# vpc-ccg/tksm

Measured on AMD Instinct MI355X. Metric: sequenced reads/s, higher is better.
Workload: dtype u8; 1 GPU; Bulk molecules, Badread error+qual model (nanopore2020, identity 84,99,5.5), 24 x 128 Mb random genome, FASTQ; kind=bulk, mean_len=1000, length_distribution=normal(1000, 200), compute_qual=True, contexts_in_flight_per_gpu=3

## Files before the change

### tksm_amd/csrc/kernels.hip

```cpp
#include "kernels.h"
#include "loop_filter.h"
#include <type_traits>

namespace tk {

#define DEV __device__ __forceinline__

constexpr int BIG = 1 << 28;
DEV bool is_inf(int v) { return v >= (1 << 27); }

struct Ph4 { uint32_t x, y, z, w; };
enum { ST_ID = 0, ST_PAD = 1, ST_IDENT = 2, ST_DRAW = 3, ST_ALNPOS = 4, ST_QUAL = 5, ST_TAIL = 6 };

DEV Ph4 philox(uint64_t seed, uint64_t read, uint32_t stream, uint32_t n) {
    uint32_t c0 = (uint32_t)read, c1 = (uint32_t)(read >> 32), c2 = stream, c3 = n;
    uint32_t k0 = (uint32_t)seed, k1 = (uint32_t)(seed >> 32);
#pragma unroll
    for (int r = 0; r < 10; r++) {
        const unsigned long long p0 = (unsigned long long)0xD2511F53u * c0, p1 = (unsigned long long)0xCD9E8D57u * c2;
        const uint32_t h0 = (uint32_t)(p0 >> 32), l0 = (uint32_t)p0, h1 = (uint32_t)(p1 >> 32), l1 = (uint32_t)p1;
        uint32_t n0 = h1 ^ c1 ^ k0, n2 = h0 ^ c3 ^ k1;
        c0 = n0; c1 = l1; c2 = n2; c3 = l0;
        k0 += 0x9E3779B9u; k1 += 0xBB67AE85u;
    }
    return Ph4{c0, c1, c2, c3};
}

DEV uint8_t base_char(int code) { return (uint8_t)((0x54474341u >> (8 * (code & 3))) & 0xff); }
DEV int code_of(uint8_t c) { return c == 'A' ? 0 : c == 'C' ? 1 : c == 'G' ? 2 : c == 'T' ? 3 : -1; }
DEV uint8_t upper(uint8_t c) { return (c >= 'a' && c <= 'z') ? (uint8_t)(c - 32) : c; }
DEV uint8_t comp(uint8_t c) {
    return c == 'A' ? 'T' : c == 'C' ? 'G' : c == 'G' ? 'C' : c == 'T' ? 'A' : c;
}

template <int CTRL, int ROW_MASK> DEV int dpp_mov(int old, int src) { return __builtin_amdgcn_update_dpp(old, src, CTRL, ROW_MASK, 0xf, false); }
constexpr int DPP_WAVE_SHL1 = 0x130, DPP_WAVE_SHR1 = 0x138;
#define TKSM_DPP_SCAN(OP, IDENT, x)                         \
    x = OP(x, dpp_mov<0x111, 0xf>(IDENT, x));               \
    x = OP(x, dpp_mov<0x112, 0xf>(IDENT, x));               \
    x = OP(x, dpp_mov<0x114, 0xf>(IDENT, x));               \
    x = OP(x, dpp_mov<0x118, 0xf>(IDENT, x));               \
    x = OP(x, dpp_mov<0x142, 0xa>(IDENT, x));               \
    x = OP(x, dpp_mov<0x143, 0xc>(IDENT, x));
DEV int scan_min_incl(int x, int) { TKSM_DPP_SCAN(min, 0x7fffffff, x) return x; }
DEV int scan_max_incl(int x, int) { TKSM_DPP_SCAN(max, (int)0x80000000, x) return x; }
DEV int add_i32(int a, int b) { return a + b; }
DEV int scan_add_incl(int x, int) { TKSM_DPP_SCAN(add_i32, 0, x) return x; }
DEV uint32_t scan_umax_incl(uint32_t x) {
#define TKSM_UMAX_STEP(C, R) x = max(x, (uint32_t)dpp_mov<C, R>(0, (int)x));
    TKSM_UMAX_STEP(0x111, 0xf) TKSM_UMAX_STEP(0x112, 0xf) TKSM_UMAX_STEP(0x114, 0xf) TKSM_UMAX_STEP(0x118, 0xf) TKSM_UMAX_STEP(0x142, 0xa) TKSM_UMAX_STEP(0x143, 0xc)
#undef TKSM_UMAX_STEP
    return x;
}
DEV int prefix_small(int v, int& total) {
    const unsigned long long b0 = __ballot(v & 1), b1 = __ballot(v & 2), b2 = __ballot(v & 4);
    const int e0 = (int)__builtin_amdgcn_mbcnt_hi((uint32_t)(b0 >> 32), __builtin_amdgcn_mbcnt_lo((uint32_t)b0, 0u));
    const int e1 = (int)__builtin_amdgcn_mbcnt_hi((uint32_t)(b1 >> 32), __builtin_amdgcn_mbcnt_lo((uint32_t)b1, 0u));
    const int e2 = (int)__builtin_amdgcn_mbcnt_hi((uint32_t)(b2 >> 32), __builtin_amdgcn_mbcnt_lo((uint32_t)b2, 0u));
    total = __popcll(b0) + 2 * __popcll(b1) + 4 * __popcll(b2);
    return e0 + 2 * e1 + 4 * e2;
}

DEV void wave_sync() {
    __builtin_amdgcn_fence(__ATOMIC_RELEASE, "wavefront");
    __builtin_amdgcn_wave_barrier();
    __builtin_amdgcn_fence(__ATOMIC_ACQUIRE, "wavefront");
}

DEV uint32_t lo32(unsigned long long v) { return (uint32_t)v; }
DEV uint32_t hi32(unsigned long long v) { return (uint32_t)(v >> 32); }
DEV unsigned long long mk64(uint32_t hi, uint32_t lo) { return ((unsigned long long)hi << 32) | lo; }
DEV uint32_t alignbit(uint32_t hi, uint32_t lo, uint32_t s) { return __builtin_amdgcn_alignbit(hi, lo, s); }
constexpr uint32_t TA = 0xF0u, TB = 0xCCu, TC = 0xAAu;
#define BOOL3(expr) ((uint32_t)((expr) & 0xFFu))
template <uint32_t TT> DEV uint32_t bool3(uint32_t x, uint32_t y, uint32_t z) { return __builtin_amdgcn_bitop3_b32(x, y, z, TT); }
template <uint32_t TT> DEV unsigned long long bool3(unsigned long long x, unsigned long long y, unsigned long long z) {
    return mk64(bool3<TT>(hi32(x), hi32(y), hi32(z)), bool3<TT>(lo32(x), lo32(y), lo32(z)));
}
DEV unsigned long long funnel128(unsigned long long x0, unsigned long long x1, int s) {
    const bool a = (s & 32) != 0;
    const uint32_t b = (uint32_t)s & 31u;
    const uint32_t y0 = a ? hi32(x0) : lo32(x0), y1 = a ? lo32(x1) : hi32(x0), y2 = a ? hi32(x1) : lo32(x1);
    return mk64(alignbit(y2, y1, b), alignbit(y1, y0, b));
}

DEV double sqrt_inrange(double x) {
    const double y = __builtin_amdgcn_rsq(x);
    double g = x * y, h = 0.5 * y;
    const double r = __builtin_fma(-h, g, 0.5);
    g = __builtin_fma(g, r, g); h = __builtin_fma(h, r, h);
    double d = __builtin_fma(-g, g, x);
    g = __builtin_fma(d, h, g);
    d = __builtin_fma(-g, g, x);
    return __builtin_fma(d, h, g);
}
DEV double rcp_refined(double b) {
    double y = __builtin_amdgcn_rcp(b);
    double r = __builtin_fma(-b, y, 1.0);
    y = __builtin_fma(y, r, y);
    r = __builtin_fma(-b, y, 1.0);
    return __builtin_fma(y, r, y);
}
DEV double div_inrange(double a, double b, double yb) {
    const double q = a * yb;
    const double r = __builtin_fma(-b, q, a);
    return __builtin_fma(r, yb, q);
}

DEV uint8_t ref_base(const RefView& R, uint64_t g) {
// ... 843 lines not shown
            dirty |= code < 0;
            const unsigned long long lo = __ballot(valid && (code & 1)), hi = __ballot(valid && (code & 2));
            if (lane == q - q0) { mylo = lo; myhi = hi; }
        }
        if (q0 + lane < fw_r) { ulonglong2 v; v.x = mylo; v.y = myhi; *reinterpret_cast<ulonglong2*>(fpl + 2 * (q0 + lane)) = v; }
    }
    const bool slow = __ballot(dirty) != 0ull;
    if (lane == 0) {
        ReadState S;
        S.errors = 0.0; S.target = target; S.est = 0.0; S.change_count = 0; S.n_base = 0; S.aln_no = 0;
        S.resume_src = -1; S.resume_j = 0; S.stage = 0; S.pending = 0; S.slow = slow ? 1 : 0; S.early = 0;
        S.st_draws = 0; S.st_aligns = 0; S.job = 0; S.raw_len = raw_len; S.res_mt = 0; S.res_cols = 0; S.res_fail = 0; S.pad3 = 0;
        FB.state[r] = S;
        O.status[r] |= status;
        if (slow) { const uint32_t idx = atomicAdd(&FB.counters[CNT_SLOW], 1u); FB.slow_list[idx] = (uint32_t)r; }
        else if (FB.early_hist) atomicAdd(&FB.early_hist[(blockIdx.x & 63u) * 256u + early_bin(L, target)], 1u);
    }
}

DEV void finish_read(const BatchView& B, const SimParams& P, const SimBuffers& O, uint64_t r, int raw_len, int out_len,
                     double identity, uint32_t status, int st_draws, int st_changes, int st_aligns, int L, int st_newlen,
                     int st_strim, int st_etrim, double errors, double target, int lane) {
    if (lane != 0) return;
    if (O.tail_len && !P.quirk_perfect) raw_len -= (int)O.tail_len[r];
    const long long h = pct_hundredths(identity);
    const uint32_t idl = B.ids[2 * r + 1];
    uint64_t rec = 1 + 36 + 8 + ndigits((unsigned)out_len) + 19 + ndigits((unsigned)raw_len) + 15 +
                   ndigits((unsigned long long)(h / 100)) + 3 + 14 + idl + 1;
    rec += (uint64_t)out_len + 1;
    if (P.fastq) rec += 2 + (uint64_t)out_len + 1;
    O.out_len[r] = (uint32_t)out_len;
    O.identity[r] = identity;
    O.rec_len[r] = rec;
    O.status[r] |= status;
    if (O.istats) {
        int32_t* s = O.istats + 16 * r;
        s[0] = st_draws; s[1] = st_changes; s[2] = st_aligns; s[3] = L; s[4] = st_newlen;
        s[5] = st_strim; s[6] = st_etrim; s[7] = (int32_t)status;
        O.dstats[2 * r] = errors; O.dstats[2 * r + 1] = target;
    }
}

DEV uint32_t draw_slot(const uint4& A, int jj) {
    const uint32_t w = (jj >> 1) == 0 ? A.x : (jj >> 1) == 1 ? A.y : (jj >> 1) == 2 ? A.z : A.w;
    return (w >> (16 * (jj & 1))) & 0xffffu;
}

DEV uint32_t planar1(uint32_t a) { return (a & 1u) | ((a >> 1) << 5); }
DEV uint32_t planar2(uint32_t a, uint32_t b) { return (a & 1u) | ((b & 1u) << 1) | ((a >> 1) << 5) | ((b >> 1) << 6); }
DEV uint4 random_change_enc(int kidx, int k, uint32_t type, uint32_t pos, uint32_t base4, uint32_t side, uint32_t r3) {
    uint32_t e[8];
#pragma unroll
    for (int j = 0; j < 8; j++) {
        const uint32_t kc = j < k ? (uint32_t)(kidx >> (2 * (k - 1 - j))) & 3u : 0u;
        uint32_t v = (1u << 12) | planar1(kc);
        if ((uint32_t)j == pos)
            v = type == 0 ? 0x8000u | (1u << 12) | planar1((kc + r3) & 3u)
              : type == 1 ? 0x8000u | (2u << 12) | (side ? planar2(kc, base4) : planar2(base4, kc))
                          : 0x8000u;
        e[j] = j < k ? v : 0u;
    }
    return make_uint4(e[0] | (e[1] << 16), e[2] | (e[3] << 16), e[4] | (e[5] << 16), e[6] | (e[7] << 16));
}

struct SlotEval { uint32_t am, lens; uint32_t e[4]; };
DEV SlotEval eval_draw(const uint16_t* nb, int k, int i, const uint4& A, bool acc) {
    SlotEval r;
    r.am = 0; r.lens = 0;
    r.e[0] = A.x | 0x80008000u; r.e[1] = A.y | 0x80008000u; r.e[2] = A.z | 0x80008000u; r.e[3] = A.w | 0x80008000u;
    if (acc) {
#pragma unroll
        for (int jj = 0; jj < 8; jj++) {
            if (jj < k) {
                const uint32_t e = draw_slot(A, jj);
                if ((e >> 15) && (nb[i + jj] & 0x8000u) == 0) r.am |= 1u << jj;
                r.lens |= ((e >> 12) & 7u) << (3 * jj);
            }
        }
    }
    return r;
}

DEV int joined_len(const uint16_t* nb, int p0, int n, int lane) {
    int m = 0;
    for (int q = 0; q < n; q += 64) {
        const int p = q + lane;
        const int len = p < n ? slot_len(nb[p0 + p]) : 0;
        int total;
        (void)prefix_small(len, total);
        m += total;
    }
    return m;
}

DEV void join_out(const uint8_t* frag, const uint16_t* nb, int n, uint8_t* out_seq, int lo, int hi, int lane) {
    int base = 0;
    for (int q = 0; q < n; q += 64) {
        const int p = q + lane;
        uint32_t code = 0; int len = 0; uint8_t orig = 0;
        if (p < n) { code = nb[p]; len = slot_len(code); orig = frag[p]; }
        int total;
        const int off = base + prefix_small(len, total);
        const uint32_t syms = code ? code & 0x3ffu : planar1((uint32_t)orig);
        for (int x2 = 0; x2 < len; x2++) { const int c = off + x2; if (c >= lo && c < hi) out_seq[c - lo] = base_char((int)(((syms >> x2) & 1u) | (((syms >> (5 + x2)) & 1u) << 1))); }
        base += total;
    }
}

#ifndef TKSM_LOOP_N
#define TKSM_LOOP_N 16
#define TKSM_LOOP_K 3
#endif
constexpr int LOOP_N = TKSM_LOOP_N, LOOP_K = TKSM_LOOP_K;
__global__ __launch_bounds__(64) __attribute__((amdgpu_num_vgpr(128))) void k_loop(ErrModelView EM, SimParams P, FastBuffers FB, const uint32_t* __restrict__ order,
                                              uint32_t begin, uint32_t count, int Wl, int from_jobs, uint32_t c0, uint32_t c1) {
#ifndef TKSM_ABLATE
    __builtin_amdgcn_s_setprio(2);
#endif
    uint32_t* lf = reinterpret_cast<uint32_t*>(lds_raw);
    const int lane = threadIdx.x;
    const uint32_t widx = blockIdx.x * 64u + (uint32_t)lane;
    bool act = widx < count;
    uint32_t r = 0, rc = 0;
    if (act) {
        if (!from_jobs) { r = order[begin + widx]; rc = (begin + widx) / FB.rs; }
        else {
            const uint32_t target = FB.prefix[c0] + widx;
            uint32_t lo2 = c0, hi2 = c1 - 1;
            while (lo2 < hi2) { const uint32_t mid = (lo2 + hi2 + 1) >> 1; if (FB.prefix[mid] <= target) lo2 = mid; else hi2 = mid - 1; }
            r = FB.prev_meta[4ull * (FB.base_prev[lo2] + (target - FB.prefix[lo2]))];
            rc = lo2;
        }
    }
    ReadState* sp = FB.state + r;
    ReadState S{};
    if (act) S = *sp;
    act = act && S.stage == 0 && !S.slow && !S.early;
    const int k = EM.k;
    const int L = S.raw_len + 2 * k;
    const uint32_t* f2 = frag2_row(FB, r);
    for (int w = 0; w < Wl; w += 16) {
        uint4 v[4];
#pragma unroll
        for (int q = 0; q < 4; q++) v[q] = *reinterpret_cast<const uint4*>(f2 + min(w + 4 * q, Wl - 4));
#pragma unroll
        for (int q = 0; q < 4; q++) {
            const int ww = min(w + 4 * q, Wl - 4);
            lf[(ww + 0) * 64 + lane] = v[q].x; lf[(ww + 1) * 64 + lane] = v[q].y; lf[(ww + 2) * 64 + lane] = v[q].z; lf[(ww + 3) * 64 + lane] = v[q].w;
        }
    }
    uint32_t* lfb = lf + (size_t)Wl * 64;
    {
        uint4 v[4];
#pragma unroll
        for (int q = 0; q < 4; q++) v[q] = EM.pt0b[q * 64 + lane];
#pragma unroll
        for (int q = 0; q < 4; q++) *reinterpret_cast<uint4*>(lfb + 4 * (q * 64 + lane)) = v[q];
    }
    __syncthreads();
    const uint16_t* lfe = reinterpret_cast<const uint16_t*>(lfb);
    uint16_t* gnb = nb_row(FB, r);
    const uint64_t g = P.first_read + (uint64_t)r * P.stride;
    const double frag_len = (double)L, target = S.target;
    const double rcp_len = rcp_refined(act ? frag_len : 1.0);
    double errors = S.errors;
    int change_count = S.change_count;
    uint32_t n = S.n_base, aln_no = S.aln_no;
    int resume_j = S.resume_j, st_draws = S.st_draws;
    double est_keep = S.est;
    if (act && S.pending == 1) {
        const uint32_t mt = S.res_mt, cols = S.res_cols;
        if (S.res_fail) {
            sp->slow = 1;
            atomicAdd(&FB.counters[CNT_EXIT + EXIT_BAND_LOOP], 1u);
            FB.slow_list[atomicAdd(&FB.counters[CNT_SLOW], 1u)] = r;
            act = false;
        } else {
            const double ident = cols ? (double)mt / (double)cols : 0.0;
            if (L <= 1000) errors = (1.0 - ident) * frag_len;
            else {
                const double estimated = (1.0 - ident) * frag_len;
                const double weight = 1000.0 / frag_len;
                errors = estimated * weight + errors * (1.0 - weight);
            }
            aln_no++;
        }
    }
    const uint32_t kmer_range = (uint32_t)(L - k);
    const long long loop_limit = 100ll * L;
    const uint32_t kmask = (1u << (2 * k)) - 1u;
    int cc25 = change_count % 25;
    enum { RUN = 0, NEED_ALN = 1, DONE = 2, IDLE = 3 };
    int st = act ? RUN : IDLE;
#ifdef TKSM_ABLATE
    if (P.ablate == 33) st = IDLE;
#endif
    const bool use_tab = EM.type != 0 && EM.alt0_noop;
    while (__ballot(st == RUN) != 0ull) {
        if (st != RUN) continue;
        const uint32_t navail = (uint32_t)max(0ll, min((long long)LOOP_N, loop_limit - (long long)n));
        uint32_t mask = 0u;
        {
            uint32_t dwv[LOOP_N], kxv[LOOP_N];
#pragma unroll
            for (int b = 0; b < LOOP_N; b++) {
                const Ph4 d = philox(P.seed, g, ST_DRAW, n + (uint32_t)b);
                const int di1 = (int)__umulhi(d.x, kmer_range);
                dwv[b] = d.y;
                const int w = di1 >> 4, o = di1 & 15;
#ifdef TKSM_ABLATE
                const bool abl_lds = P.ablate == 35 || P.ablate == 36;
                const uint32_t hi = (abl_lds || w < Wl) ? lf[min(w, Wl - 1) * 64 + lane] : f2[w], lo = (abl_lds || w + 1 < Wl) ? lf[min(w + 1, Wl - 1) * 64 + lane] : f2[w + 1];
#else
                const uint32_t hi = w < Wl ? lf[w * 64 + lane] : f2[w], lo = w + 1 < Wl ? lf[(w + 1) * 64 + lane] : f2[w + 1];
#endif
                kxv[b] = (uint32_t)(mk64(hi, lo) >> (64 - 2 * o - 2 * k)) & kmask;
            }
            uint32_t ev[LOOP_N];
#pragma unroll
            for (int b = 0; b < LOOP_N; b++) ev[b] = lfe[tklf::loop_filter_key(kxv[b])];
            uint32_t sure = 0u, und = 0u;
#pragma unroll
            for (int b = 0; b < LOOP_N; b++) {
                const int c = tklf::loop_filter_classify(ev[b], dwv[b]);
                sure |= c == tklf::DRAW_CHANGE ? 1u << b : 0u;
                und |= c == tklf::DRAW_UNDECIDED ? 1u << b : 0u;
            }
            if (!use_tab) { sure = (1u << LOOP_N) - 1u; und = 0u; }
#ifdef TKSM_ABLATE
            const bool abl_t0 = P.ablate == 34 || P.ablate == 36;
            if (abl_t0 && use_tab) { sure = 0u; und = (1u << LOOP_N) - 1u; }
#endif
            uint32_t t0v[LOOP_N];
#pragma unroll
            for (int b = 0; b < LOOP_N; b++) {
                const uint32_t off = (und >> b) & 1u ? kxv[b] << 2 : 0u;
#ifdef TKSM_ABLATE
                t0v[b] = abl_t0 ? 0xCF000000u : *reinterpret_cast<const uint32_t*>(reinterpret_cast<const char*>(EM.pt0) + off);
#else
                t0v[b] = *reinterpret_cast<const uint32_t*>(reinterpret_cast<const char*>(EM.pt0) + off);
#endif
            }
#pragma unroll
            for (int b = 0; b < LOOP_N; b++) mask |= !(dwv[b] < t0v[b]) ? 1u << b : 0u;
            mask = (sure | (und & mask)) & ((1u << navail) - 1u);
        }
        int di[LOOP_K], kidx[LOOP_K];
        uint32_t bj[LOOP_K], dw[LOOP_K];
        bool rest;
        {
            uint32_t mm = mask;
#pragma unroll
            for (int j = 0; j < LOOP_K; j++) {
                bj[j] = mm ? (uint32_t)__builtin_ctz(mm) : (uint32_t)LOOP_N;
                mm &= mm - 1u;
                const uint32_t bb = min(bj[j], (uint32_t)LOOP_N - 1u);
                const Ph4 d = philox(P.seed, g, ST_DRAW, n + bb);
                dw[j] = d.y;
                di[j] = (int)__umulhi(d.x, kmer_range);
                const int w = di[j] >> 4, o = di[j] & 15;
                const uint32_t hi = w < Wl ? lf[w * 64 + lane] : f2[w], lo = w + 1 < Wl ? lf[(w + 1) * 64 + lane] : f2[w + 1];
                kidx[j] = (int)((uint32_t)(mk64(hi, lo) >> (64 - 2 * o - 2 * k)) & kmask);
            }
            rest = mm != 0u;
        }
        int cls[LOOP_K];
        uint4 seg[LOOP_K];
        int nab[LOOP_K];
#pragma unroll
        for (int j = 0; j < LOOP_K; j++) { seg[j] = EM.pseg[kidx[j]]; nab[j] = EM.max_alts; }
        if (!EM.uniform_nalts) {
#pragma unroll
            for (int j = 0; j < LOOP_K; j++) nab[j] = (int)EM.nalts[kidx[j]];
        }
        int sbase[LOOP_K];
        uint4 th0[LOOP_K], th1[LOOP_K];
        struct __attribute__((packed, aligned(4))) W5 { uint32_t v[5]; };
        W5 nbw[LOOP_K];
#pragma unroll
        for (int j = 0; j < LOOP_K; j++) {
            const bool have = bj[j] < (uint32_t)LOOP_N;
            cls[j] = !have ? 0 : EM.type == 0 ? 2 : (dw[j] < seg[j].x ? (EM.alt0_noop ? 0 : 3) : 1);
            sbase[j] = 8 * ((dw[j] < seg[j].y ? 0 : 1) + (dw[j] < seg[j].z ? 0 : 1) + (dw[j] < seg[j].w ? 0 : 1));
            const uint4* c4 = reinterpret_cast<const uint4*>(EM.cdf32 + (cls[j] == 1 ? (size_t)kidx[j] * 32 + sbase[j] : (size_t)0));
            th0[j] = c4[0]; th1[j] = c4[1];
            const uint16_t* gp = cls[j] != 0 ? gnb + (di[j] & ~1) : FB.st_nb;
            nbw[j] = *reinterpret_cast<const W5*>(gp);
        }
        uint4 alt[LOOP_K];
#pragma unroll
        for (int j = 0; j < LOOP_K; j++) {
            size_t at = 0;
            if (cls[j] == 1 || cls[j] == 3) {
                const int na = nab[j];
                int a2 = 0;
                if (cls[j] == 1) {
                    const uint32_t w = dw[j];
                    a2 = sbase[j];
                    a2 += !(w < th0[j].x) ? 1 : 0; a2 += !(w < th0[j].y) ? 1 : 0; a2 += !(w < th0[j].z) ? 1 : 0; a2 += !(w < th0[j].w) ? 1 : 0;
                    a2 += !(w < th1[j].x) ? 1 : 0; a2 += !(w < th1[j].y) ? 1 : 0; a2 += !(w < th1[j].z) ? 1 : 0; a2 += !(w < th1[j].w) ? 1 : 0;
                    a2 = min(a2, na);
                }
                if (a2 == na) cls[j] = 2;
                else if (a2 == 0 && EM.alt0_noop) cls[j] = 0;
                else at = (size_t)kidx[j] * EM.max_alts + a2;
            }
            alt[j] = EM.alts_enc[at];
        }
        const uint32_t n0 = n;
        const uint32_t end = rest ? bj[LOOP_K - 1] + 1u : navail;
        uint32_t wrote = 0u;
        auto top_of_iteration = [&](double& est) -> bool {
            est = 1.0 - div_inrange(errors, frag_len, rcp_len);
            if ((double)change_count > 0.9 * frag_len || est <= target) { st = DONE; st_draws = (int)n; return false; }
            if ((long long)n + 1 > loop_limit) { st = DONE; st_draws = (int)loop_limit; return false; }
            return true;
        };
#pragma unroll
        for (int j = 0; j <= LOOP_K; j++) {
            if (st != RUN) break;
            double est = est_keep;
            if (j == LOOP_K || bj[j] >= (uint32_t)LOOP_N) {
                if (n - n0 < end) { if (!top_of_iteration(est)) break; n = n0 + end; }
                if (!rest && navail < (uint32_t)LOOP_N) (void)top_of_iteration(est);
                break;
            }
            if (resume_j == 0 && !top_of_iteration(est)) break;
            n = n0 + bj[j];
            if (cls[j] != 0) {
                uint4 A = alt[j];
                if (cls[j] == 2) {
                    const Ph4 d2 = philox(P.seed, g, ST_DRAW, n0 + bj[j]);
                    const uint32_t dzj = d2.z, dvj = d2.w;
                    const uint32_t type = __umulhi(dzj, 3u), pos = __umulhi(dvj, (uint32_t)k);
                    const uint32_t base4 = dvj & 3u, side = (dvj >> 2) & 1u;
                    const uint32_t r3 = (((dzj & 0xffffu) * 3u) >> 16) + 1u;
                    const uint32_t kc = ((uint32_t)kidx[j] >> (2 * (k - 1 - (int)pos))) & 3u;
                    const uint32_t v = type == 0 ? 0x8000u | (1u << 12) | planar1((kc + r3) & 3u)
                                     : type == 1 ? 0x8000u | (2u << 12) | (side ? planar2(kc, base4) : planar2(base4, kc))
                                                 : 0x8000u;
                    const uint32_t w = v << (16 * (pos & 1u)), which = pos >> 1;
                    A = make_uint4(which == 0 ? w : 0u, which == 1 ? w : 0u, which == 2 ? w : 0u, which == 3 ? w : 0u);
                }
                uint32_t dm = ((A.x >> 15) & 1u) | ((A.x >> 31) << 1) | (((A.y >> 15) & 1u) << 2) | ((A.y >> 31) << 3) |
                              (((A.z >> 15) & 1u) << 4) | ((A.z >> 31) << 5) | (((A.w >> 15) & 1u) << 6) | ((A.w >> 31) << 7);
                dm &= ((1u << k) - 1u) & ~((1u << resume_j) - 1u);
                if (dm) {
                    bool stale = false;
#pragma unroll
                    for (int j2 = 0; j2 < LOOP_K; j2++) if (j2 < j) stale |= ((wrote >> j2) & 1u) && abs(di[j] - di[j2]) < k;
                    if (stale) nbw[j] = *reinterpret_cast<const W5*>(gnb + (di[j] & ~1));
                    const double f15 = est * sqrt_inrange(est);
                    const int odd = di[j] & 1;
                    int stop_at = -1;
                    while (dm) {
                        const int jj = __builtin_ctz(dm);
                        dm &= dm - 1u;
                        const int ent = jj + odd, wi = ent >> 1;
                        const uint32_t cw2 = wi == 0 ? nbw[j].v[0] : wi == 1 ? nbw[j].v[1] : wi == 2 ? nbw[j].v[2] : wi == 3 ? nbw[j].v[3] : nbw[j].v[4];
                        if (((cw2 >> (16 * (ent & 1))) & 0x8000u) == 0u) {
                            const uint32_t e = draw_slot(A, jj);
                            gnb[di[j] + jj] = (uint16_t)(e | 0x8000u);
                            wrote |= 1u << j;
                            change_count++;
                            const int len_j = (int)((e >> 12) & 7u);
                            errors += (double)(len_j < 2 ? 1 : len_j - 1) * f15;
                            if (++cc25 == 25) { cc25 = 0; stop_at = jj; dm = 0u; }
                        }
                    }
                    if (stop_at >= 0) {
                        st = NEED_ALN;
                        if (stop_at + 1 < k) { resume_j = stop_at + 1; est_keep = est; }
                        else { resume_j = 0; n++; }
                        break;
                    }
                }
            }
            resume_j = 0;
            n++;
        }
    }
    int st_aligns = S.st_aligns;
    uint32_t job = 0;
    {
        bool need = st == NEED_ALN;
        unsigned long long todo = __ballot(need);
        while (todo) {
            const int leader = __builtin_ctzll(todo);
            const uint32_t lrc = (uint32_t)__shfl((int)rc, leader, 64);
            const unsigned long long grp = __ballot(need && rc == lrc);
            uint32_t base = 0;
            if (lane == leader) base = FB.base_cur[lrc] + atomicAdd(&FB.job_cnt[lrc * 32u], (uint32_t)__popcll(grp));
            base = (uint32_t)__shfl((int)base, leader, 64);
            if (need && rc == lrc) { job = base + (uint32_t)__popcll(grp & ((1ull << lane) - 1ull)); need = false; }
            todo &= ~grp;
        }
    }
    if (st == NEED_ALN) {
        st_aligns++;
        uint32_t p0 = 0, nrows = (uint32_t)L;
        if (L > 1000) {
            uint32_t r2 = r;
            asm volatile("" : "+v"(r2));
            p0 = __umulhi(philox(P.seed, P.first_read + (uint64_t)r2 * P.stride, ST_ALNPOS, aln_no).x, (uint32_t)(L - 1000 + 1));
            nrows = 1000u;
        }
        *reinterpret_cast<uint4*>(FB.job_meta + 4ull * job) = make_uint4(r, p0, nrows, 0u);
    }
    if (st == NEED_ALN || st == DONE) {
        sp->errors = errors; sp->est = est_keep; sp->change_count = change_count; sp->n_base = n; sp->aln_no = aln_no;
        sp->resume_src = -1; sp->resume_j = (int16_t)resume_j; sp->st_draws = st_draws; sp->st_aligns = st_aligns;
        sp->pending = st == NEED_ALN ? 1 : 0;
        sp->job = job;
        sp->stage = st == NEED_ALN ? 0 : 3;
        if (st == DONE) {
// ... 299 lines not shown
        const uint32_t pjob = FB.base_prev[lo2] + (target - FB.prefix[lo2]);
        r = (uint64_t)__builtin_amdgcn_readfirstlane((int)FB.prev_meta[4ull * pjob]) & 0xffffffffull;
        pos = lo2 * FB.rs;
    }
    ReadState S = FB.state[r];
    if (S.stage == 2 || S.slow) return;
    if (S.stage == 0) return;
    uint16_t* gnb = nb_row(FB, r);
    const int per_wave = STATE_IN_HBM ? lds_ncap + 128 : lds_lcap * 3 + lds_ncap + 128;
    uint8_t* lds_wave = lds_raw + (size_t)wave * per_wave;
    uint8_t* frag = STATE_IN_HBM ? frag_row(FB, r) : lds_wave;
    uint16_t* nb = STATE_IN_HBM ? gnb : reinterpret_cast<uint16_t*>(lds_wave + lds_lcap);
    uint8_t* aux = STATE_IN_HBM ? lds_wave : lds_wave + 3 * (size_t)lds_lcap;
    const int k = EM.k;
    const uint64_t g = P.first_read + r * P.stride;
    const int raw_len = __builtin_amdgcn_readfirstlane(S.raw_len);
    const int L = raw_len + 2 * k;
    const uint64_t slot = O.slot_off[r];
    const int cap = __builtin_amdgcn_readfirstlane((int)((O.slot_off[r + 1] - slot) >> 1));
    uint8_t* out_seq = O.scratch + slot;
    uint8_t* out_qual = out_seq + cap;
    if (!STATE_IN_HBM) {
        const uint8_t* gfrag0 = frag_row(FB, r);
        for (int t = lane * 4; t < L; t += 256) *reinterpret_cast<uint32_t*>(frag + t) = *reinterpret_cast<const uint32_t*>(gfrag0 + t);
        for (int t = lane * 2; t < L; t += 128) *reinterpret_cast<uint32_t*>(nb + t) = *reinterpret_cast<const uint32_t*>(gnb + t);
    }
    wave_sync();
    uint32_t status = 0;
    const double frag_len = (double)L;
    const double errors = S.errors;
    const double target = S.target;
    const int change_count = __builtin_amdgcn_readfirstlane(S.change_count), st_draws = __builtin_amdgcn_readfirstlane(S.st_draws);
    int st_aligns = __builtin_amdgcn_readfirstlane(S.st_aligns);
    double identity = 1.0;

    int start_trim, end_trim;
    {
        int v1 = lane < k ? slot_len(nb[lane]) : 0, v2 = lane < k ? slot_len(nb[L - k + lane]) : 0;
        (void)prefix_small(v1, start_trim);
        (void)prefix_small(v2, end_trim);
    }
    const int jcap = min(lds_ncap, cap);
    const int m = joined_len(nb, 0, L, lane);
    int lo = start_trim, hi = end_trim == 0 ? 0 : m - end_trim;
    lo = min(lo, m); hi = max(hi, lo);
    if (m > jcap) { status |= 1; lo = hi = 0; }
    const int out_len = hi - lo;
    const bool want_q = P.compute_q && m > 0 && !(status & 1);
    if (want_q) {
        const uint32_t mt = S.res_mt, cols = S.res_cols, fail = S.res_fail;
        if (fail) { go_slow(FB, r, lane, EXIT_BAND_ERR); return; }
        identity = cols ? (double)mt / (double)cols : 0.0;
        const uint32_t rc1 = pos / FB.rs;
        const uint8_t* gp = FB.prev_popd + FB.geo_prev[rc1].popd_off + (size_t)(S.job - FB.base_prev[rc1]) * FB.geo_prev[rc1].ncap;
        wave_sync();
        uint8_t* popd = aux + 16;
        for (int t = lane; t < m; t += 64) popd[t] = gp[t];
        wave_sync();
        const int margins = (QM.kmer_size - 1) / 2;
        const uint32_t hmask = (uint32_t)QM.n_slots - 1u;
        for (int i2 = lo + lane; i2 < hi; i2 += 64) {
#ifdef TKSM_ABLATE
            if (P.ablate == 40) { out_qual[i2 - lo] = 40; continue; }
#endif
            const int d = max(0, max(margins - i2, i2 + margins - (m - 1)));
            int row = -1; uint32_t roff = 0, rcnt = 0;
            auto probe = [&](uint64_t key) {
                uint32_t sl = (uint32_t)qs_hash(key) & hmask;
#ifdef TKSM_ABLATE
                if (P.ablate == 41) { row = (int)(sl & 1023u); roff = 0u; rcnt = 1u; return; }
#endif
                for (;;) {
                    const uint4 e = QM.ent[sl];
                    const uint64_t kk = ((uint64_t)e.y << 32) | e.x;
                    if (kk == key) { row = (int)sl; roff = e.z; rcnt = e.w; break; }
                    if (kk == 0) break;
                    sl = (sl + 1) & hmask;
                }
            };
            if (margins <= 4) {
                const int ob = 16 + i2 - 4, sh = ob & 3;
                const uint32_t* aw = reinterpret_cast<const uint32_t*>(aux) + (ob >> 2);
                const uint32_t w0 = aw[0], w1 = aw[1], w2 = aw[2];
                const uint32_t b0 = __builtin_amdgcn_alignbyte(w1, w0, sh), b1 = __builtin_amdgcn_alignbyte(w2, w1, sh), b2 = w2 >> (8 * sh);
                auto byte_at = [&](int j) -> uint32_t { return j < 4 ? (b0 >> (8 * j)) & 255u : j < 8 ? (b1 >> (8 * (j - 4))) & 255u : b2 & 255u; };
                uint64_t K[5]; int ln[5];
                K[0] = byte_at(4) & 3u; ln[0] = 1;
#pragma unroll
                for (int h = 1; h <= 4; h++) {
                    const uint32_t bl = byte_at(4 - h);
                    const int ddl = (int)(bl >> 2), ddr = (int)(byte_at(3 + h) >> 2);
                    ln[h] = ln[h - 1] + 2 + ddl + ddr;
                    const bool fits = ln[h] <= 29;
                    const int sl_ = fits ? 2 * (1 + ddl) : 0, sr_ = fits ? 2 * (1 + ddl + ln[h - 1]) : 0, so_ = fits ? 2 * (ln[h] - 1) : 0;
                    const int dl2 = fits ? 2 * ddl : 0, dr2 = fits ? 2 * ddr : 0;
                    K[h] = (uint64_t)(bl & 3u) | (((1ull << dl2) - 1ull) << 2) | (K[h - 1] << sl_) | (((1ull << dr2) - 1ull) << sr_) |
                           ((uint64_t)(byte_at(4 + h) & 3u) << so_);
                }
                const int hmax = margins - d;
                bool pend = true;
#pragma unroll
                for (int h = 4; h >= 0; h--) {
                    const bool tryit = pend && h <= hmax;
                    if (__ballot(tryit) == 0ull) continue;
                    if (tryit && ln[h] <= 29) { probe(K[h] | ((uint64_t)ln[h] << 58)); pend = row < 0; }
#ifdef TKSM_ABLATE
                    if (P.ablate == 44) { if (row < 0) row = (int)(K[h] & 1023u); pend = false; }
                    if (P.ablate == 45 && h == 3) { if (row < 0) row = (int)(K[h] & 1023u); pend = false; }
#endif
                }
            } else {
                int s0 = i2 - margins + d, e0 = i2 + margins - d;
                for (;;) {
                    uint64_t key = 0; int len = 0; bool ok = true;
                    for (int x2 = s0; x2 <= e0; x2++) {
                        if (x2 > s0) {
                            const int dd = popd[x2 - 1] >> 2;
                            if (len + dd > 29) { ok = false; break; }
                            key |= ((1ull << (2 * dd)) - 1ull) << (2 * len); len += dd;
                        }
                        if (len >= 29) { ok = false; break; }
                        key |= (uint64_t)(popd[x2] & 3) << (2 * len); len++;
                    }
                    if (ok) probe(key | ((uint64_t)len << 58));
                    if (row >= 0 || s0 == e0) break;
                    s0++; e0--;
                }
            }
            uint8_t q = 0;
#ifdef TKSM_ABLATE
            if (P.ablate == 42) { out_qual[i2 - lo] = (uint8_t)(33 + (row & 31)); continue; }
            if (P.ablate == 43 && row >= 0) {
                const uint32_t w = (uint32_t)i2 * 2654435761u;
                const uint32_t a2 = QM.guide[(size_t)row * 64 + (w >> 26)] & 0x7fu;
                out_qual[i2 - lo] = (uint8_t)(33 + QM.pairs[roff + min(a2, rcnt - 1u)].y); continue;
            }
#endif
            if (row >= 0) {
                const uint32_t w = philox(P.seed, g, ST_QUAL, (uint32_t)i2).x;
                uint32_t a2 = QM.guide[(size_t)row * 64 + (w >> 26)];
                if (QM.guide_direct && (a2 & 0x80u)) q = (uint8_t)(a2 & 0x7fu);
                else {
                    uint2 pr = QM.pairs[roff + a2];
                    while (a2 + 1 < rcnt && !(w < pr.x)) { a2++; pr = QM.pairs[roff + a2]; }
                    q = (uint8_t)pr.y;
                }
            }
            out_qual[i2 - lo] = (uint8_t)(q + 33);
        }
    } else {
        identity = 1.0 - errors / frag_len;
    }
    join_out(frag, nb, L, out_seq, lo, hi, lane);
    if (P.quirk_perfect) identity = 1.0;
    finish_read(B, P, O, r, P.quirk_perfect ? out_len : raw_len, out_len, identity, status, st_draws, change_count, st_aligns, L, m,
                start_trim, end_trim, errors, target, lane);
    if (lane == 0) FB.state[r].stage = 2;
}

__global__ void k_collect_unfinished(FastBuffers FB, uint64_t n_reads) {
    const uint64_t r = (uint64_t)blockIdx.x * blockDim.x + threadIdx.x;
    if (r >= n_reads) return;
    ReadState S = FB.state[r];
    if (S.stage != 2 && !S.slow) {
        FB.state[r].slow = 1;
        const uint32_t idx = atomicAdd(&FB.counters[CNT_SLOW], 1u);
        FB.slow_list[idx] = (uint32_t)r;
    }
}

DEV uint32_t range_of_job(const FastBuffers& FB, uint32_t job0) {
    uint32_t rng = 0, hi2 = FB.n_ranges - 1;
    while (rng < hi2) { const uint32_t mid = (rng + hi2 + 1) >> 1; if (FB.base_cur[mid] <= job0) rng = mid; else hi2 = mid - 1; }
    return rng;
}
__global__ __launch_bounds__(64) void k_qjobs(FastBuffers FB, int k, uint32_t count) {
    const int lane = threadIdx.x;
    const uint32_t widx = blockIdx.x * 64u + (uint32_t)lane;
    bool need = widx < count;
    uint32_t r = 0, rc = 0, job = 0;
    if (need) { const uint2 e = FB.defer_list[widx]; r = e.x; rc = e.y; }
    need = need && FB.state[r].stage == 3 && !FB.state[r].slow;
    const bool mine = need;
    unsigned long long todo = __ballot(need);
    while (todo) {
        const int leader = __builtin_ctzll(todo);
        const uint32_t lrc = (uint32_t)__shfl((int)rc, leader, 64);
        const unsigned long long grp = __ballot(need && rc == lrc);
        uint32_t base = 0;
        if (lane == leader) base = FB.base_cur[lrc] + atomicAdd(&FB.job_cnt[lrc * 32u], (uint32_t)__popcll(grp));
        base = (uint32_t)__shfl((int)base, leader, 64);
        if (need && rc == lrc) { job = base + (uint32_t)__popcll(grp & ((1ull << lane) - 1ull)); need = false; }
        todo &= ~grp;
    }
    if (mine) {
        ReadState* sp = FB.state + r;
        const uint32_t L = (uint32_t)(sp->raw_len + 2 * k);
        *reinterpret_cast<uint4*>(FB.job_meta + 4ull * job) = make_uint4(r, 0u, L | 0x80000000u, 0u);
        sp->resume_src = -1; sp->pending = 1; sp->stage = 1; sp->job = job;
    }
}

DEV int wave_max(int v) {
#pragma unroll
    for (int o = 32; o > 0; o >>= 1) v = max(v, __shfl_xor(v, o, 64));
    return v;
}
DEV void list_append(uint32_t* list, uint32_t* counter, bool want, uint32_t job, int lane) {
    const unsigned long long wm = __ballot(want);
    if (!wm) return;
    uint32_t base = 0;
    if (lane == 0) base = atomicAdd(counter, (uint32_t)__popcll(wm));
    base = __shfl(base, 0, 64);
    if (want) list[base + (uint32_t)__popcll(wm & ((1ull << lane) - 1ull))] = job;
}


constexpr uint32_t ENT_EMPTY = 0xF0000000u;
constexpr int BACKLOG_DRAIN = 20;
struct AlnJobF {
    bool act; int p0, n;
    const uint16_t* nb;
// ... 993 lines not shown
```

Before: 15.68 million reads/s.

## Use bitop3 XOR in Philox, flat SWAR quality keys, and cheaper join loops

Adds a templated Philox that emits the three-input XOR through the gfx950 bitop3 intrinsic from a chosen round onward, used for draw and quality RNG. Replaces the nested per-level quality-key construction with a SWAR byte-prefix flat key builder that takes 32-bit, 64-bit or a nested fallback path chosen per wave. Simplifies joined_len to one strided accumulation plus a single wave scan, and unrolls the join_out per-slot writes with a ballot guard. These aim to cut ALU work in hot RNG, quality and join code, at the cost of more code paths and subtle key-equivalence risk.

```diff
diff --git a/tksm_amd/csrc/kernels.hip b/tksm_amd/csrc/kernels.hip
--- a/tksm_amd/csrc/kernels.hip
+++ b/tksm_amd/csrc/kernels.hip
@@ -1,5 +1,6 @@
 #include "kernels.h"
 #include "loop_filter.h"
+#include "qs_keys.h"
 #include <type_traits>
 
 namespace tk {
@@ -12,19 +13,23 @@
 struct Ph4 { uint32_t x, y, z, w; };
 enum { ST_ID = 0, ST_PAD = 1, ST_IDENT = 2, ST_DRAW = 3, ST_ALNPOS = 4, ST_QUAL = 5, ST_TAIL = 6 };
 
-DEV Ph4 philox(uint64_t seed, uint64_t read, uint32_t stream, uint32_t n) {
+template <int LANE_FROM>
+DEV Ph4 philox_t(uint64_t seed, uint64_t read, uint32_t stream, uint32_t n) {
     uint32_t c0 = (uint32_t)read, c1 = (uint32_t)(read >> 32), c2 = stream, c3 = n;
     uint32_t k0 = (uint32_t)seed, k1 = (uint32_t)(seed >> 32);
 #pragma unroll
     for (int r = 0; r < 10; r++) {
         const unsigned long long p0 = (unsigned long long)0xD2511F53u * c0, p1 = (unsigned long long)0xCD9E8D57u * c2;
         const uint32_t h0 = (uint32_t)(p0 >> 32), l0 = (uint32_t)p0, h1 = (uint32_t)(p1 >> 32), l1 = (uint32_t)p1;
-        uint32_t n0 = h1 ^ c1 ^ k0, n2 = h0 ^ c3 ^ k1;
+        uint32_t n0, n2;
+        if (r >= LANE_FROM) { n0 = __builtin_amdgcn_bitop3_b32(h1, c1, k0, 0x96u); n2 = __builtin_amdgcn_bitop3_b32(h0, c3, k1, 0x96u); }
+        else { n0 = h1 ^ c1 ^ k0; n2 = h0 ^ c3 ^ k1; }
         c0 = n0; c1 = l1; c2 = n2; c3 = l0;
         k0 += 0x9E3779B9u; k1 += 0xBB67AE85u;
     }
     return Ph4{c0, c1, c2, c3};
 }
+DEV Ph4 philox(uint64_t seed, uint64_t read, uint32_t stream, uint32_t n) { return philox_t<10>(seed, read, stream, n); }
 
 DEV uint8_t base_char(int code) { return (uint8_t)((0x54474341u >> (8 * (code & 3))) & 0xff); }
 DEV int code_of(uint8_t c) { return c == 'A' ? 0 : c == 'C' ? 1 : c == 'G' ? 2 : c == 'T' ? 3 : -1; }
@@ -1034,15 +1039,9 @@
 }
 
 DEV int joined_len(const uint16_t* nb, int p0, int n, int lane) {
-    int m = 0;
-    for (int q = 0; q < n; q += 64) {
-        const int p = q + lane;
-        const int len = p < n ? slot_len(nb[p0 + p]) : 0;
-        int total;
-        (void)prefix_small(len, total);
-        m += total;
-    }
-    return m;
+    int acc = 0;
+    for (int p = lane; p < n; p += 64) acc += slot_len(nb[p0 + p]);
+    return __builtin_amdgcn_readlane(scan_add_incl(acc, 0), 63);
 }
 
 DEV void join_out(const uint8_t* frag, const uint16_t* nb, int n, uint8_t* out_seq, int lo, int hi, int lane) {
@@ -1054,7 +1053,13 @@
         int total;
         const int off = base + prefix_small(len, total);
         const uint32_t syms = code ? code & 0x3ffu : planar1((uint32_t)orig);
-        for (int x2 = 0; x2 < len; x2++) { const int c = off + x2; if (c >= lo && c < hi) out_seq[c - lo] = base_char((int)(((syms >> x2) & 1u) | (((syms >> (5 + x2)) & 1u) << 1))); }
+        auto sym_char = [&](int x2) { return base_char((int)(((syms >> x2) & 1u) | (((syms >> (5 + x2)) & 1u) << 1))); };
+        uint8_t* const dst = out_seq + (off - lo);
+        if (len >= 1 && off >= lo && off < hi) dst[0] = sym_char(0);
+        if (__ballot(len >= 2) != 0ull) {
+#pragma unroll
+            for (int x2 = 1; x2 < 5; x2++) { const int c = off + x2; if (x2 < len && c >= lo && c < hi) dst[x2] = sym_char(x2); }
+        }
         base += total;
     }
 }
@@ -1156,7 +1161,7 @@
             uint32_t dwv[LOOP_N], kxv[LOOP_N];
 #pragma unroll
             for (int b = 0; b < LOOP_N; b++) {
-                const Ph4 d = philox(P.seed, g, ST_DRAW, n + (uint32_t)b);
+                const Ph4 d = philox_t<3>(P.seed, g, ST_DRAW, n + (uint32_t)b);
                 const int di1 = (int)__umulhi(d.x, kmer_range);
                 dwv[b] = d.y;
                 const int w = di1 >> 4, o = di1 & 15;
@@ -1207,7 +1212,7 @@
                 bj[j] = mm ? (uint32_t)__builtin_ctz(mm) : (uint32_t)LOOP_N;
                 mm &= mm - 1u;
                 const uint32_t bb = min(bj[j], (uint32_t)LOOP_N - 1u);
-                const Ph4 d = philox(P.seed, g, ST_DRAW, n + bb);
+                const Ph4 d = philox_t<3>(P.seed, g, ST_DRAW, n + bb);
                 dw[j] = d.y;
                 di[j] = (int)__umulhi(d.x, kmer_range);
                 const int w = di[j] >> 4, o = di[j] & 15;
@@ -1282,7 +1287,7 @@
             if (cls[j] != 0) {
                 uint4 A = alt[j];
                 if (cls[j] == 2) {
-                    const Ph4 d2 = philox(P.seed, g, ST_DRAW, n0 + bj[j]);
+                    const Ph4 d2 = philox_t<3>(P.seed, g, ST_DRAW, n0 + bj[j]);
                     const uint32_t dzj = d2.z, dvj = d2.w;
                     const uint32_t type = __umulhi(dzj, 3u), pos = __umulhi(dvj, (uint32_t)k);
                     const uint32_t base4 = dvj & 3u, side = (dvj >> 2) & 1u;
@@ -1748,28 +1753,20 @@
                 const int ob = 16 + i2 - 4, sh = ob & 3;
                 const uint32_t* aw = reinterpret_cast<const uint32_t*>(aux) + (ob >> 2);
                 const uint32_t w0 = aw[0], w1 = aw[1], w2 = aw[2];
-                const uint32_t b0 = __builtin_amdgcn_alignbyte(w1, w0, sh), b1 = __builtin_amdgcn_alignbyte(w2, w1, sh), b2 = w2 >> (8 * sh);
-                auto byte_at = [&](int j) -> uint32_t { return j < 4 ? (b0 >> (8 * j)) & 255u : j < 8 ? (b1 >> (8 * (j - 4))) & 255u : b2 & 255u; };
+                uint32_t b0 = __builtin_amdgcn_alignbyte(w1, w0, sh), b1 = __builtin_amdgcn_alignbyte(w2, w1, sh), b2 = w2 >> (8 * sh);
+                const int hmax = margins - d;
+                if (__ballot(hmax < 4) != 0ull) tkqk::qs_window_trim(b0, b1, b2, 4 - hmax);
+                const tkqk::QsWindow qw = tkqk::qs_window(b0, b1, b2);
                 uint64_t K[5]; int ln[5];
-                K[0] = byte_at(4) & 3u; ln[0] = 1;
-#pragma unroll
-                for (int h = 1; h <= 4; h++) {
-                    const uint32_t bl = byte_at(4 - h);
-                    const int ddl = (int)(bl >> 2), ddr = (int)(byte_at(3 + h) >> 2);
-                    ln[h] = ln[h - 1] + 2 + ddl + ddr;
-                    const bool fits = ln[h] <= 29;
-                    const int sl_ = fits ? 2 * (1 + ddl) : 0, sr_ = fits ? 2 * (1 + ddl + ln[h - 1]) : 0, so_ = fits ? 2 * (ln[h] - 1) : 0;
-                    const int dl2 = fits ? 2 * ddl : 0, dr2 = fits ? 2 * ddr : 0;
-                    K[h] = (uint64_t)(bl & 3u) | (((1ull << dl2) - 1ull) << 2) | (K[h - 1] << sl_) | (((1ull << dr2) - 1ull) << sr_) |
-                           ((uint64_t)(byte_at(4 + h) & 3u) << so_);
-                }
-                const int hmax = margins - d;
+                if (__ballot(tkqk::qs_window_span(qw) != tkqk::QS_SPAN_32) == 0ull) tkqk::qs_keys(qw, tkqk::QS_SPAN_32, K, ln);
+                else if (__ballot(qw.wide) == 0ull) tkqk::qs_keys(qw, tkqk::QS_SPAN_64, K, ln);
+                else tkqk::qs_keys(qw, tkqk::QS_SPAN_WIDE, K, ln);
                 bool pend = true;
 #pragma unroll
                 for (int h = 4; h >= 0; h--) {
                     const bool tryit = pend && h <= hmax;
                     if (__ballot(tryit) == 0ull) continue;
-                    if (tryit && ln[h] <= 29) { probe(K[h] | ((uint64_t)ln[h] << 58)); pend = row < 0; }
+                    if (tryit && ln[h] <= tkqk::QS_MAX_OPS) { probe(tkqk::qs_probe_key(K[h], ln[h])); pend = row < 0; }
 #ifdef TKSM_ABLATE
                     if (P.ablate == 44) { if (row < 0) row = (int)(K[h] & 1023u); pend = false; }
                     if (P.ablate == 45 && h == 3) { if (row < 0) row = (int)(K[h] & 1023u); pend = false; }
@@ -1803,7 +1800,7 @@
             }
 #endif
             if (row >= 0) {
-                const uint32_t w = philox(P.seed, g, ST_QUAL, (uint32_t)i2).x;
+                const uint32_t w = philox_t<4>(P.seed, g, ST_QUAL, (uint32_t)i2).x;
                 uint32_t a2 = QM.guide[(size_t)row * 64 + (w >> 26)];
                 if (QM.guide_direct && (a2 & 0x80u)) q = (uint8_t)(a2 & 0x7fu);
                 else {
diff --git a/tksm_amd/csrc/qs_keys.h b/tksm_amd/csrc/qs_keys.h
--- /dev/null
+++ b/tksm_amd/csrc/qs_keys.h
@@ -0,0 +1,95 @@
+#pragma once
+#include <stdint.h>
+
+#if defined(__HIPCC__)
+#define TKQK_HD __host__ __device__ inline
+#define TKQK_UNROLL _Pragma("unroll")
+#else
+#define TKQK_HD inline
+#define TKQK_UNROLL
+#endif
+
+namespace tkqk {
+
+constexpr int QS_MAX_OPS = 29;
+constexpr int QS_FLAT32_OPS = 15;
+
+struct QsWindow {
+    uint32_t b0, b1, b2;
+    uint32_t pa, pb;
+    bool wide;
+    int ln4;
+};
+
+TKQK_HD void qs_window_trim(uint32_t& b0, uint32_t& b1, uint32_t& b2, int z) {
+    if (z <= 0) return;
+    b0 = z >= 4 ? 0u : b0 & (0xffffffffu << (8 * z));
+    b1 = b1 & (0x03ffffffu >> (8 * (z - 1)));
+    b2 = 0u;
+}
+
+TKQK_HD uint32_t qs_byte_prefix(uint32_t s) { s += s << 8; return s + (s << 16); }
+
+TKQK_HD QsWindow qs_window(uint32_t b0, uint32_t b1, uint32_t b2) {
+    QsWindow w;
+    w.b0 = b0; w.b1 = b1; w.b2 = b2 & 255u;
+    w.pa = qs_byte_prefix(((b0 >> 2) & 0x3f3f3f3fu) + 0x01010101u);
+    w.pb = qs_byte_prefix(((b1 >> 2) & 0x3f3f3f3fu) + 0x01010101u + (w.pa >> 24));
+    w.wide = ((b0 | b1) & 0x80808080u) != 0u || w.pb - 0x01000000u >= ((uint32_t)(QS_MAX_OPS - 1) << 24);
+    w.ln4 = (int)(w.pb >> 24) + 1;
+    return w;
+}
+
+template <class W>
+TKQK_HD void qs_keys_flat(const QsWindow& w, uint64_t K[5], int ln[5]) {
+    const uint32_t n0 = ~w.b0 & 0x03030303u, n1 = ~w.b1 & 0x03030303u, n2 = ~w.b2 & 3u;
+    const uint32_t sa = w.pa << 1, sb = w.pb << 1;
+    W x = (W)(n0 & 255u);
+    x |= (W)((n0 >> 8) & 255u) << (sa & 255u);
+    x |= (W)((n0 >> 16) & 255u) << ((sa >> 8) & 255u);
+    x |= (W)(n0 >> 24) << ((sa >> 16) & 255u);
+    x |= (W)(n1 & 255u) << (sa >> 24);
+    x |= (W)((n1 >> 8) & 255u) << (sb & 255u);
+    x |= (W)((n1 >> 16) & 255u) << ((sb >> 8) & 255u);
+    x |= (W)(n1 >> 24) << ((sb >> 16) & 255u);
+    x |= (W)n2 << (sb >> 24);
+    x = ~x;
+    const uint32_t rev = ((w.pa >> 16) & 0xffu) | (w.pa & 0xff00u) | ((w.pa & 0xffu) << 16);
+    const uint32_t lens = w.pb - rev + 0x01010101u, sh = rev << 1;
+    K[0] = w.b1 & 3u; ln[0] = 1;
+    TKQK_UNROLL
+    for (int h = 1; h <= 4; h++) {
+        const uint32_t l = (lens >> (8 * (h - 1))) & 255u, s = (sh >> (8 * (h - 1))) & 255u;
+        ln[h] = (int)l;
+        K[h] = (uint64_t)((x >> s) & (((W)1 << (2 * l)) - (W)1));
+    }
+}
+
+TKQK_HD void qs_keys_nested(uint32_t b0, uint32_t b1, uint32_t b2, uint64_t K[5], int ln[5]) {
+    auto byte_at = [&](int j) -> uint32_t { return j < 4 ? (b0 >> (8 * j)) & 255u : j < 8 ? (b1 >> (8 * (j - 4))) & 255u : b2 & 255u; };
+    K[0] = byte_at(4) & 3u; ln[0] = 1;
+    TKQK_UNROLL
+    for (int h = 1; h <= 4; h++) {
+        const uint32_t bl = byte_at(4 - h);
+        const int ddl = (int)(bl >> 2), ddr = (int)(byte_at(3 + h) >> 2);
+        ln[h] = ln[h - 1] + 2 + ddl + ddr;
+        const bool fits = ln[h] <= 29;
+        const int sl_ = fits ? 2 * (1 + ddl) : 0, sr_ = fits ? 2 * (1 + ddl + ln[h - 1]) : 0, so_ = fits ? 2 * (ln[h] - 1) : 0;
+        const int dl2 = fits ? 2 * ddl : 0, dr2 = fits ? 2 * ddr : 0;
+        K[h] = (uint64_t)(bl & 3u) | (((1ull << dl2) - 1ull) << 2) | (K[h - 1] << sl_) | (((1ull << dr2) - 1ull) << sr_) |
+               ((uint64_t)(byte_at(4 + h) & 3u) << so_);
+    }
+}
+
+enum { QS_SPAN_32 = 0, QS_SPAN_64 = 1, QS_SPAN_WIDE = 2 };
+TKQK_HD int qs_window_span(const QsWindow& w) { return w.wide ? QS_SPAN_WIDE : w.ln4 > QS_FLAT32_OPS ? QS_SPAN_64 : QS_SPAN_32; }
+
+TKQK_HD void qs_keys(const QsWindow& w, int span, uint64_t K[5], int ln[5]) {
+    if (span == QS_SPAN_32) qs_keys_flat<uint32_t>(w, K, ln);
+    else if (span == QS_SPAN_64) qs_keys_flat<uint64_t>(w, K, ln);
+    else qs_keys_nested(w.b0, w.b1, w.b2, K, ln);
+}
+
+TKQK_HD uint64_t qs_probe_key(uint64_t k, int ln) { return k | ((uint64_t)ln << 58); }
+
+}
```

Result: faster. 15.94 million reads/s (median of 6 runs) (+1.6%).
